# tenpy/cyten

Hardware: AMD Instinct MI355X
Metric: block-sparse tdot+SVD GFLOP/s (fp64) (higher is better)
Workload: dtype f64

## Files before the change

cyten_amd/csrc/blocked_qr.h:

```cpp
#pragma once
#include "common.h"

namespace cyb {

constexpr int NBK = 32;

struct BqrMat {
    double* Ac;
    int64_t ld;
    int32_t m, n, k;
    double* V;
    double* T;
    double* tau;
    double* scratch;
    int64_t scr_half;
    int32_t v_zeroed = 0;
    double* ctl = nullptr;
    double* parts = nullptr;
    double stop_rel2 = 0.0;
    int32_t reflect_always = 0;
};

size_t bqr_aux_bytes(int64_t m, int64_t n, int64_t ld, int64_t kc);
size_t bqr_carve(BqrMat& q, char* base, int64_t kc);

int bqr_strip_slots(int64_t rows);

int bqr_factor(cyb_ctx_t ctx, const std::vector<BqrMat>& mats);

struct BqrTarget {
    int32_t mat;
    double* C;
    int64_t ldc;
    int32_t kc;
};
int bqr_apply_q(cyb_ctx_t ctx, const std::vector<BqrMat>& mats, const std::vector<BqrTarget>& targets);

struct XposeDesc {
    const double* in;
    double* out;
    int64_t ldi, ldo;
    int32_t R, C, upper, rlim;
    int32_t plain, pad;
};
int xpose_batched(cyb_ctx_t ctx, const std::vector<XposeDesc>& descs);
struct EyeDesc {
    double* C;
    int64_t ld;
    int32_t m, kc;
    int32_t col0, pad;
};
int eye_cols_batched(cyb_ctx_t ctx, const std::vector<EyeDesc>& descs);

}
```

cyten_amd/csrc/blocked_qr.hip:

```cpp
#include "blocked_qr.h"

#include <algorithm>
#include <cstdlib>
#include <utility>

namespace cyb {
namespace {

#define GLOBAL_AS __attribute__((address_space(1)))
typedef GLOBAL_AS double* gp;
typedef const GLOBAL_AS double* gcp;
typedef double d4 __attribute__((ext_vector_type(4)));

constexpr int PNT = 512;
constexpr int PNW = PNT / 64;

__device__ __forceinline__ double wave_sum(double v)
{
#pragma unroll
    for (int o = 32; o > 0; o >>= 1) v += __shfl_xor(v, o);
    return v;
}

struct PanelDesc {
// ... 859 lines not shown
            }
        }
    }
    if constexpr (LA) {
        if (d.next_off) {
            asm volatile("s_waitcnt vmcnt(0)" ::: "memory");
            __syncthreads();
            if (tid == 0) {
                __builtin_amdgcn_fence(__ATOMIC_RELEASE, "agent");
                __hip_atomic_store(la_flags + (d.next_off - 1), la_tag, __ATOMIC_RELAXED, __HIP_MEMORY_SCOPE_AGENT);
            }
        }
    }
    if constexpr (FUSE_PANEL) {
        __shared__ PanelShared psh;
        if (d.next_off) {
            __syncthreads();
            const PanelDesc pd = *reinterpret_cast<const PanelDesc*>(reinterpret_cast<const char*>(descs) + d.next_off);
            panel_reg_body<RP_RPT_FUSED>(pd, psh, tid);
        }
    }
}

struct ChunkDesc {
    double* C;
    const double* V;
    const double* T;
    double* wpart;
    int64_t ldc, ldv;
    int32_t mr, nc, pw, transT;
    int32_t slot, n_slots, row0, step;
    const double* ctl;
    double* part_out;
};

__global__ void __launch_bounds__(ST_NT) strip_w1_kernel(const ChunkDesc* __restrict__ descs)
{
    __shared__ double part[ST_NW][NBK][ST_LS];
    const ChunkDesc d = descs[blockIdx.x];
    if (d.ctl) {
        const double stopped = *(gcp)d.ctl;
        if (stopped != 0.0 && (double)d.step >= stopped - 1.0) return;
    }
    const int tid = threadIdx.x, lane = tid & 63, wave = tid >> 6;
    const int x = lane & 15, kq = lane >> 4;
    gcp V = (gcp)d.V;
// ... 178 lines not shown
            for (int o = 32; o > 0; o >>= 1) nrm2 += __shfl_xor(nrm2, o);
            __syncthreads();
            if (lane == 0) W1s[0][wave] = nrm2;
            __syncthreads();
            if (tid == 0) {
                double t = 0.0;
#pragma unroll
                for (int w = 0; w < ST_NW; ++w) t += W1s[0][w];
                *(gp)d.part_out = t;
            }
        }
    }
}

inline size_t al256(size_t b) { return (b + 255) / 256 * 256; }

__global__ void __launch_bounds__(256) xpose_kernel(const XposeDesc* __restrict__ descs)
{
    __shared__ double tile[32][33];
    const XposeDesc d = descs[blockIdx.y];
    gcp in = (gcp)d.in;
    gp out = (gp)d.out;
    const int tx = threadIdx.x & 31, ty = threadIdx.x >> 5;
    if (d.plain) {
        const int64_t tot = (int64_t)d.R * d.C;
        for (int64_t e = (int64_t)blockIdx.x * 256 + threadIdx.x; e < tot; e += (int64_t)gridDim.x * 256) {
            const int64_t r = e / d.C, c = e % d.C;
            out[r * d.ldo + c] = in[r * d.ldi + c];
        }
        return;
    }
    const int tr = (d.R + 31) / 32, tc = (d.C + 31) / 32;
    for (int t = blockIdx.x; t < tr * tc; t += gridDim.x) {
        const int r0 = (t / tc) * 32, c0 = (t % tc) * 32;
        __syncthreads();
#pragma unroll
        for (int q = 0; q < 4; ++q) {
            const int c = c0 + ty + 8 * q, r = r0 + tx;
            tile[ty + 8 * q][tx] = (c < d.C && r < d.R) ? in[(int64_t)c * d.ldi + r] : 0.0;
        }
        __syncthreads();
#pragma unroll
        for (int q = 0; q < 4; ++q) {
            const int r = r0 + ty + 8 * q, c = c0 + tx;
            if (r < d.R && c < d.C) {
                double v = tile[tx][ty + 8 * q];
                if (d.upper && (r > c || r >= d.rlim)) v = 0.0;
                out[(int64_t)r * d.ldo + c] = v;
            }
        }
    }
}

__global__ void __launch_bounds__(256) eye_cols_kernel(const EyeDesc* __restrict__ descs)
{
    const EyeDesc d = descs[blockIdx.y];
    gp C = (gp)d.C;
    const int64_t tot = (int64_t)d.m * d.kc;
    for (int64_t e = (int64_t)blockIdx.x * 256 + threadIdx.x; e < tot; e += (int64_t)gridDim.x * 256) {
        const int64_t c = e / d.m, i = e % d.m;
        C[c * d.ld + i] = (i == c + d.col0) ? 1.0 : 0.0;
    }
}

}

int xpose_batched(cyb_ctx_t ctx, const std::vector<XposeDesc>& descs)
{
    if (descs.empty()) return CYB_OK;
    void* d = nullptr;
    CYB_TRY(ctx->upload(descs.data(), sizeof(XposeDesc) * descs.size(), &d));
    hipLaunchKernelGGL(xpose_kernel, dim3(helper_grid_x(descs.size()), (unsigned)descs.size()), dim3(256), 0, ctx->stream, static_cast<const XposeDesc*>(d));
    CYB_HIP(hipGetLastError());
// ... 462 lines not shown
    }
    if (last_rest >= 0) CYB_HIP(hipStreamWaitEvent(ctx->stream, ctx->ev_pool[2 * (size_t)last_rest + 1], 0));
    if (la_used) {
        unsigned int h_err = 0;
        CYB_HIP(hipMemcpyAsync(&h_err, la_flags + la_err, sizeof(unsigned int), hipMemcpyDeviceToHost, ctx->stream));
        CYB_HIP(hipStreamSynchronize(ctx->stream));
        if (h_err) {
            set_error("blocked QR: a look-ahead panel workgroup waited more than a second for its strip");
            return CYB_ERR_HIP;
        }
    }
    if (multi) {
        unsigned int h_err = 0;
        CYB_HIP(hipMemcpyAsync(&h_err, xbase + t_bytes, sizeof(unsigned int), hipMemcpyDeviceToHost, ctx->stream));
        CYB_HIP(hipStreamSynchronize(ctx->stream));
        if (h_err) {
            set_error("blocked QR: a workgroup of the multi-workgroup panel kernel waited more than a second for its partners");
            return CYB_ERR_HIP;
        }
    }
    return CYB_OK;
}

int bqr_apply_q(cyb_ctx_t ctx, const std::vector<BqrMat>& mats, const std::vector<BqrTarget>& targets)
{
    int max_pan = 0;
    for (const auto& t : targets) max_pan = std::max(max_pan, (mats[(size_t)t.mat].k + NBK - 1) / NBK);
    const bool strips = use_strips();
    struct Step {
        GemmStaged s1, s3;
        size_t off_sd = 0;
        unsigned n_sd = 0;
        size_t off_cd = 0;
        unsigned n_cd = 0;
    };
    const bool split = strips && strip_split_mode() != 0;
    double* wsplit = nullptr;
    if (split) {
        size_t n_ch = 0;
        for (const auto& t : targets) n_ch += (size_t)((t.kc + NBK - 1) / NBK) * (size_t)bqr_strip_slots(mats[(size_t)t.mat].m);
        void* w = nullptr;
        CYB_TRY(ctx->workspace(sizeof(double) * NBK * NBK * std::max<size_t>(n_ch, 1), &w, 4));
        wsplit = static_cast<double*>(w);
    }
    std::vector<Step> steps;
    std::vector<char> image;
    int chunk = 2;
    for (int c0 = max_pan - 1; c0 >= 0; c0 -= chunk, chunk *= 3) {
    const int c1 = std::max(-1, c0 - chunk);
    steps.clear();
    image.clear();
    for (int p = c0; p > c1; --p) {
        GemmBatch g1, g3;
        std::vector<StripDesc> sd;
        for (const auto& t : targets) {
            const BqrMat& q = mats[(size_t)t.mat];
            const int j0 = p * NBK;
            if (j0 >= q.k || t.kc <= 0) continue;
            const int pw = std::min(NBK, q.k - j0);
            const int64_t mr = q.m - j0;
            double* W1 = q.scratch + q.scr_half;
            CYB_REQUIRE((int64_t)NBK * t.kc <= q.scr_half, "bqr_apply_q: target wider than the carved scratch");
            const double* Vp = q.V + (size_t)j0 * q.ld + j0;
            double* Ct = t.C + j0;
            const double* Tp = q.T + (size_t)p * NBK * NBK;
            if (strips) {
                const size_t s_begin = sd.size();
                add_strips(sd, Ct, t.ldc, t.kc, Vp, q.ld, Tp, mr, pw, 0);
                if (q.ctl && q.stop_rel2 > 0.0)
                    for (size_t si = s_begin; si < sd.size(); ++si) {
                        sd[si].ctl = q.ctl;
                        sd[si].step = p;
                    }
                continue;
            }
            const int ns = w_split(mr);
            const int64_t chunk = ((mr + ns - 1) / ns + 15) / 16 * 16;
            const int32_t seg0 = (int32_t)g3.segs.size();
            for (int sidx = 0; sidx < ns; ++sidx) {
                const int64_t r0 = chunk * sidx, rows = std::min(chunk, mr - r0);
                if (rows <= 0) break;
                double* W2s = W1 + (size_t)sidx * q.scr_half;
                g1.add_post(W2s, pw, t.kc, t.kc, Vp + r0, q.ld, 1, Ct + r0, 1, t.ldc, rows, 1.0, 0.0, Tp, NBK, 1);
                g3.segs.push_back(cyb_gemm_seg{W2s, Vp, pw, 1, t.kc, q.ld, 1});
            }
            g3.probs.push_back(cyb_gemm_prob{Ct, t.kc, mr, t.ldc, seg0, (int32_t)g3.segs.size(), -1.0, 1.0});
        }
        if (g1.empty() && sd.empty()) continue;
        Step st;
        if (!g1.empty()) {
            CYB_TRY(g1.stage(ctx, image, st.s1));
            CYB_TRY(g3.stage(ctx, image, st.s3));
        }
        if (!sd.empty()) {
            sort_strips(sd);
            st.n_sd = (unsigned)sd.size();
            const size_t off = (image.size() + 255) / 256 * 256;
            image.resize(off + sizeof(StripDesc) * sd.size());
            memcpy(image.data() + off, sd.data(), sizeof(StripDesc) * sd.size());
            st.off_sd = off;
            std::vector<std::pair<int, int>> cnt;
            for (const auto& d : sd) cnt.push_back({d.mr, 1});
            const int step_ch = split ? choose_chunk_rows(cnt, ctx->n_cu) : 0;
            if (step_ch > 0) {
                std::vector<ChunkDesc> cd;
                make_chunks(sd, wsplit, step_ch, cd);
                st.n_cd = (unsigned)cd.size();
                const size_t offc = (image.size() + 255) / 256 * 256;
                image.resize(offc + sizeof(ChunkDesc) * cd.size());
                memcpy(image.data() + offc, cd.data(), sizeof(ChunkDesc) * cd.size());
                st.off_cd = offc;
            }
        }
        steps.push_back(st);
    }
    if (steps.empty()) continue;
    void* d_image = nullptr;
    CYB_TRY(ctx->upload(image.data(), image.size(), &d_image));
    for (const auto& st : steps) {
        if (st.n_cd) {
            const ChunkDesc* cdp = reinterpret_cast<const ChunkDesc*>(static_cast<char*>(d_image) + st.off_cd);
            hipLaunchKernelGGL(strip_w1_kernel, dim3(st.n_cd), dim3(ST_NT), 0, ctx->stream, cdp);
            hipLaunchKernelGGL(strip_apply_kernel<false>, dim3(st.n_cd), dim3(ST_NT), 0, ctx->stream, cdp);
            CYB_HIP(hipGetLastError());
        } else if (st.n_sd) {
            hipLaunchKernelGGL(reflector_strip_kernel<false>, dim3(st.n_sd), dim3(ST_NT), 0, ctx->stream,
                               reinterpret_cast<const StripDesc*>(static_cast<char*>(d_image) + st.off_sd), (int)st.n_sd,
                               static_cast<const PanelDesc*>(nullptr), static_cast<unsigned int*>(nullptr), 0u, 0);
            CYB_HIP(hipGetLastError());
        }
        CYB_TRY(gemm_launch_staged(ctx, st.s1, d_image));
        CYB_TRY(gemm_launch_staged(ctx, st.s3, d_image));
    }
    }
    return CYB_OK;
}

}
```

cyten_amd/csrc/svd_jacobi.hip:

```cpp
#include "blocked_qr.h"
#include "jacobi_engine.h"

#include <algorithm>
#include <cmath>
#include <cstdlib>

namespace cyb {
namespace {

#define GLOBAL_AS __attribute__((address_space(1)))
typedef GLOBAL_AS double* gp;
typedef const GLOBAL_AS double* gcp;

struct PrepDesc {
    const double* A;
    int64_t lda;
    int32_t m, n;
    double* W;
    double* J;
    int32_t nvp, lenp;
    int32_t transpose;
    int32_t pad;
    const double* shift;
};
// ... 90 lines not shown
    const double* sig_lq = nullptr;
};

__global__ void __launch_bounds__(256) row_norm_kernel(const PostDesc* __restrict__ descs)
{
    const PostDesc d = descs[blockIdx.y];
    gcp W = (gcp)d.W;
    const int lane = threadIdx.x & 63;
    for (int j = blockIdx.x * 4 + (threadIdx.x >> 6); j < d.nv; j += gridDim.x * 4) {
        double s = 0.0;
        for (int c = lane; c < d.len; c += 64) {
            const double v = W[(int64_t)j * d.lenp + c];
            s += v * v;
        }
#pragma unroll
        for (int o = 32; o > 0; o >>= 1) s += __shfl_xor(s, o);
        if (lane == 0) {
            const double o = d.sig_lq ? ((gcp)d.sig_lq)[j] : 0.0;
            ((gp)d.sig)[j] = (o > 0.0 && s > 0.0) ? o : sqrt(s);
        }
    }
}

__global__ void __launch_bounds__(256) rank_kernel(const PostDesc* __restrict__ descs)
{
    constexpr int CH = 2048;
    __shared__ double keys[CH];
    const PostDesc d = descs[blockIdx.y];
    gcp sig = (gcp)d.sig;
    const double shift = d.shift ? *(gcp)d.shift : 0.0;
    const int msk = d.cplx ? ~1 : ~0;
    const int per = (d.nv + (int)gridDim.x * 256 - 1) / ((int)gridDim.x * 256);
    for (int it = 0; it < per; ++it) {
        const int j = (it * (int)gridDim.x + (int)blockIdx.x) * 256 + (int)threadIdx.x;
        const bool mine = j < d.nv;
        const double sj = mine ? sig[j & msk] : 0.0;
        int r = 0;
        for (int k0 = 0; k0 < d.nv; k0 += CH) {
            const int kn = min(CH, d.nv - k0);
            __syncthreads();
            for (int k = threadIdx.x; k < kn; k += 256) keys[k] = sig[(k0 + k) & msk];
            __syncthreads();
            if (mine) {
                if (d.mode == 0) {
                    for (int k = 0; k < kn; ++k) {
                        const double sk = keys[k];
                        r += (sk > sj || (sk == sj && k0 + k < j)) ? 1 : 0;
                    }
                } else {
                    for (int k = 0; k < kn; ++k) {
                        const double sk = keys[k];
                        r += (sk < sj || (sk == sj && k0 + k < j)) ? 1 : 0;
                    }
                }
            }
        }
        if (mine) {
            d.rank[j] = r;
            d.S[r] = (d.mode == 0) ? sj : sj - shift;
        }
    }
}

__global__ void __launch_bounds__(256) write_factors_kernel(const PostDesc* __restrict__ descs)
{
    __shared__ double tile[32][33];
    __shared__ int rk[32];
    __shared__ double sc[32];
    const PostDesc d = descs[blockIdx.y];
    gcp W = (gcp)d.W;
    gcp J = (gcp)d.J;
    const int tx = threadIdx.x & 31, ty = threadIdx.x >> 5;
    double smax = 0.0;
    if (d.mode == 0) smax = ((gcp)d.S)[0];
    const double thresh = fmax(smax * 1e-280, 1e-300);

    const bool col_from_W = (d.mode == 1) || d.transposed;
    gcp csrc = col_from_W ? W : J;
    const int csrc_ld = col_from_W ? d.lenp : d.nvp;
    const int c_rows = col_from_W ? d.len : d.nv;
    gcp rsrc = col_from_W ? J : W;
    const int rsrc_ld = col_from_W ? d.nvp : d.lenp;
    const int r_cols = col_from_W ? d.nv : d.len;

// ... 272 lines not shown
        q.scratch = reinterpret_cast<double*>(base + o.scratch);
        q.n_null = reinterpret_cast<int32_t*>(base + o.nnull);
        q.null_scale = 0.0;
        q.cplx = cplx ? 1 : 0;
    }
    void* d_prep = nullptr;
    CYB_TRY(ctx->upload(prep.data(), sizeof(PrepDesc) * prep.size(), &d_prep));
    if (mode == 1) {
        void* d_nd = nullptr;
        CYB_TRY(ctx->upload(nd.data(), sizeof(NormDesc) * nd.size(), &d_nd));
        hipLaunchKernelGGL(fro_shift_kernel, dim3((unsigned)nmat), dim3(256), 0, st, static_cast<const NormDesc*>(d_nd));
    }
    hipLaunchKernelGGL(prep_kernel, dim3(64, (unsigned)nmat), dim3(256), 0, st, static_cast<const PrepDesc*>(d_prep));
    CYB_HIP(hipGetLastError());
    std::vector<int32_t> sweeps;
    const int jst = jacobi_orthogonalise(ctx, mats, 40, sweeps, cplx);
    if (info)
        for (int64_t b = 0; b < nmat; ++b) info[b] = sweeps[(size_t)b];
    if (jst != CYB_OK && jst != CYB_ERR_NOCONV) return jst;
    void* d_post = nullptr;
    CYB_TRY(ctx->upload(post.data(), sizeof(PostDesc) * post.size(), &d_post));
    const PostDesc* dp = static_cast<const PostDesc*>(d_post);
    hipLaunchKernelGGL(row_norm_kernel, dim3(helper_grid_x((size_t)nmat), (unsigned)nmat), dim3(256), 0, st, dp);
    hipLaunchKernelGGL(rank_kernel, dim3(8, (unsigned)nmat), dim3(256), 0, st, dp);
    hipLaunchKernelGGL(write_factors_kernel, dim3(helper_grid_x((size_t)nmat), (unsigned)nmat), dim3(256), 0, st, dp);
    if (mode == 0) hipLaunchKernelGGL(complete_null_kernel, dim3((unsigned)nmat), dim3(256), 0, st, dp);
    CYB_HIP(hipGetLastError());
    if (info) CYB_HIP(hipStreamSynchronize(st));
    return jst;
}


namespace {

struct RowsDesc {
    double* W;
    const double* sig;
    const int32_t* idx;
    double* buf;
    int32_t kp, k, cnt, pad;
    const int32_t* col;
};
__global__ void __launch_bounds__(256) gather_rows_kernel(const RowsDesc* __restrict__ descs)
{
    const RowsDesc d = descs[blockIdx.y];
    gcp W = (gcp)d.W;
    gp buf = (gp)d.buf;
// ... 228 lines not shown
#pragma unroll
        for (int o = 32; o > 0; o >>= 1) n2 += __shfl_xor(n2, o);
        if (lane == 0) ((gp)d.sigo)[d.idx[i]] = n2 > 0.0 ? f : 0.0;
        f = n2 > 0.0 ? f / sqrt(n2) : 0.0;
        for (int c = lane; c < d.kp; c += 64) Wc[(int64_t)i * d.kp + c] = c < d.k ? f * C[(int64_t)i * d.k + c] : 0.0;
    }
}

static int launch_row_moves(cyb_ctx_t ctx, const std::vector<RowMoveDesc>& v, bool jscatter = false)
{
    if (v.empty()) return CYB_OK;
    void* d = nullptr;
    CYB_TRY(ctx->upload(v.data(), sizeof(RowMoveDesc) * v.size(), &d));
    if (jscatter)
        hipLaunchKernelGGL(j_scatter_kernel, dim3(64, (unsigned)v.size()), dim3(256), 0, ctx->stream, static_cast<const RowMoveDesc*>(d));
    else
        hipLaunchKernelGGL(row_move_kernel, dim3(helper_grid_x(v.size()), (unsigned)v.size()), dim3(256), 0, ctx->stream, static_cast<const RowMoveDesc*>(d));
    CYB_HIP(hipGetLastError());
    return CYB_OK;
}

}

static int run_svd_qr(cyb_ctx_t ctx, int64_t nmat, const cyb_svd_desc* sd, int32_t* info, int flags, int32_t* rank_out)
{
    if (nmat == 0) return CYB_OK;
    const bool cplx = (flags & CYB_SVD_EMBEDDED_COMPLEX) != 0;
    hipStream_t st = ctx->stream;
    auto al = [](size_t b) { return (b + 255) / 256 * 256; };
    struct Lay {
        int m, n, k, L, kp;
        bool tall;
        size_t Ac, aux, W, J, sig, rank, thr, nnull, Cq, Fc, aux2, Cn, idx, Wc, Jc;
        size_t bad, Wq, aux3, Cq2, sig2;
        size_t stop;
        size_t sigo;
        size_t dev;
        bool lq = false;
        bool jrec = false;
        int r0 = 0;
        std::vector<int32_t> good0;
    };
    std::vector<Lay> lay((size_t)nmat);
    size_t off = 0;
    size_t sig_begin = off;
    for (int64_t b = 0; b < nmat; ++b) {
        Lay& l = lay[(size_t)b];
        l.m = (int)sd[b].m;
        l.n = (int)sd[b].n;
        l.k = std::min(l.m, l.n);
        l.L = std::max(l.m, l.n);
        l.kp = round_up(l.k, 64);
        l.tall = l.m >= l.n;
        l.sig = off;
        off += sizeof(double) * (size_t)l.kp;
    }
    for (int64_t b = 0; b < nmat; ++b) {
        lay[(size_t)b].thr = off;
        off += sizeof(double);
    }
    for (int64_t b = 0; b < nmat; ++b) {
        lay[(size_t)b].bad = off;
        off += sizeof(double);
    }
    for (int64_t b = 0; b < nmat; ++b) {
        lay[(size_t)b].dev = off;
        off += sizeof(double);
    }
    const size_t sig_bytes = off - sig_begin;
    off = al(off);
    for (int64_t b = 0; b < nmat; ++b) {
        Lay& l = lay[(size_t)b];
        auto take = [&](size_t bytes) {
            const size_t o = off;
            off += al(bytes);
            return o;
        };
        l.Ac = take(sizeof(double) * (size_t)l.L * l.k);
        l.aux = take(bqr_aux_bytes(l.L, l.k, l.L, l.k));
        l.stop = take(sizeof(double) * (size_t)(2 + (l.k + cyb::NBK - 1) / cyb::NBK * cyb::bqr_strip_slots(l.L)));
        l.W = take(sizeof(double) * (size_t)l.kp * l.kp);
        l.J = take(sizeof(double) * (size_t)l.kp * l.kp);
        l.rank = take(sizeof(int32_t) * (size_t)l.kp);
        l.nnull = take(sizeof(int32_t));
        l.Cq = take(sizeof(double) * (size_t)l.L * l.k);
        l.Fc = take(sizeof(double) * (size_t)l.k * l.k);
        l.aux2 = take(bqr_aux_bytes(l.k, l.k, l.k, l.k));
        l.Cn = take(sizeof(double) * (size_t)l.k * l.k);
        l.Wc = take(sizeof(double) * (size_t)l.kp * l.kp);
        l.Jc = take(sizeof(double) * (size_t)l.kp * l.kp);
        l.Wq = take(sizeof(double) * (size_t)l.kp * l.kp);
        l.aux3 = take(bqr_aux_bytes(l.k, l.k, l.kp, l.k));
        l.Cq2 = take(sizeof(double) * (size_t)l.k * l.k);
        l.sig2 = take(sizeof(double) * (size_t)l.kp);
        l.sigo = take(sizeof(double) * (size_t)l.kp);
    }
    const size_t idx_begin = off;
    for (int64_t b = 0; b < nmat; ++b) {
        lay[(size_t)b].idx = off;
        off += sizeof(int32_t) * (size_t)lay[(size_t)b].k;
    }
    off = al(off);
    void* ws = nullptr;
    CYB_TRY(ctx->workspace(off, &ws, 0));
    char* base = static_cast<char*>(ws);
    CYB_HIP(hipMemsetAsync(ws, 0, off, st));
    auto dp = [&](size_t o) { return reinterpret_cast<double*>(base + o); };

    std::vector<BqrMat> qm((size_t)nmat);
    std::vector<XposeDesc> x_in, x_r;
    std::vector<EyeDesc> eyeJ;
    std::vector<JMat> jm((size_t)nmat);
    for (int64_t b = 0; b < nmat; ++b) {
        const Lay& l = lay[(size_t)b];
        BqrMat& q = qm[(size_t)b];
        q.Ac = dp(l.Ac);
        q.ld = l.L;
        q.m = l.L;
        q.n = l.k;
        q.k = l.k;
        bqr_carve(q, base + l.aux, l.k);
        q.v_zeroed = 1;
        q.reflect_always = cplx ? 1 : 0;
        q.ctl = dp(l.stop);
        q.parts = dp(l.stop) + 2;
        q.stop_rel2 = ((double)l.L * 2.220446049250313e-16) * ((double)l.L * 2.220446049250313e-16);
        if (l.tall)
            x_in.push_back(XposeDesc{sd[b].A, q.Ac, sd[b].lda, l.L, l.n, l.m, 0, 0, 0, 0});
        else
            x_in.push_back(XposeDesc{sd[b].A, q.Ac, sd[b].lda, l.L, l.m, l.n, 0, 0, 1, 0});
        x_r.push_back(XposeDesc{q.Ac, dp(l.W), l.L, l.kp, l.k, l.k, 1, l.k, 0, 0});
        eyeJ.push_back(EyeDesc{dp(l.J), l.kp, l.kp, l.kp, 0, 0});
        JMat& j = jm[(size_t)b];
        j.W = dp(l.W);
        j.J = dp(l.J);
        j.nvp = l.kp;
        j.lenp = l.kp;
        j.nb = row_blocks(l.k, l.kp);
        j.nv = l.k;
        j.len = l.k;
        j.rec_j = 0;
        j.tol = 2.220446049250313e-16 * std::max(16.0, 4.0 * std::sqrt((double)l.k));
        j.thr2 = 0.0;
    }
    CYB_TRY(xpose_batched(ctx, x_in));
    CYB_TRY(bqr_factor(ctx, qm));
    CYB_TRY(xpose_batched(ctx, x_r));
    CYB_TRY(eye_cols_batched(ctx, eyeJ));
    std::vector<PostDesc> post((size_t)nmat);
    for (int64_t b = 0; b < nmat; ++b) {
        const Lay& l = lay[(size_t)b];
        PostDesc& q = post[(size_t)b];
        q.W = dp(l.W);
// ... 6 lines not shown
        q.mode = 0;
        q.sig = dp(l.sig);
        q.rank = reinterpret_cast<int32_t*>(base + l.rank);
        q.S = sd[b].S;
        q.U = l.tall ? nullptr : sd[b].U;
        q.ldu = sd[b].ldu;
        q.Vh = l.tall ? sd[b].Vh : nullptr;
        q.ldvh = sd[b].ldvh;
        q.shift = nullptr;
        q.scratch = nullptr;
        q.n_null = reinterpret_cast<int32_t*>(base + l.nnull);
        q.null_scale = 1.0;
        q.cplx = cplx ? 1 : 0;
    }
    void* d_post = nullptr;
    const PostDesc* dpost = nullptr;
    std::vector<double> h_sig(sig_bytes / sizeof(double));
    auto sig_of = [&](const Lay& l) { return h_sig.data() + (l.sig - sig_begin) / sizeof(double); };
    CYB_TRY(ctx->upload(post.data(), sizeof(PostDesc) * post.size(), &d_post));
    dpost = static_cast<const PostDesc*>(d_post);
    hipLaunchKernelGGL(row_norm_kernel, dim3(helper_grid_x((size_t)nmat), (unsigned)nmat), dim3(256), 0, st, dpost);
    CYB_HIP(hipGetLastError());
    CYB_TRY(ctx->d2h(h_sig.data(), base + sig_begin, sig_bytes));
    {
        std::vector<int32_t> idx_all;
        std::vector<size_t> idx_off((size_t)nmat, 0);
        for (int64_t b = 0; b < nmat; ++b) {
            Lay& l = lay[(size_t)b];
            const double* sg = sig_of(l);
            double fro2 = 0.0;
            for (int j = 0; j < l.k; ++j) fro2 += sg[j] * sg[j];
            const double sc = (double)l.L * 2.220446049250313e-16;
            const double thr2 = fro2 * sc * sc;
            jm[(size_t)b].thr2 = thr2;
            std::vector<int32_t> nul;
            for (int j = 0; j < l.k; ++j) {
                const double v = cplx ? std::max(sg[j & ~1], sg[std::min(j | 1, l.k - 1)]) : sg[j];
                (v * v > thr2 ? l.good0 : nul).push_back(j);
            }
            l.r0 = (int)l.good0.size();
            idx_off[(size_t)b] = idx_all.size();
            idx_all.insert(idx_all.end(), l.good0.begin(), l.good0.end());
            idx_all.insert(idx_all.end(), nul.begin(), nul.end());
        }
        static const bool no_lq = getenv("CYB_SVD_NOLQ") != nullptr;
        static const bool lq_always = getenv("CYB_SVD_LQ_ALWAYS") != nullptr;
// ... 271 lines not shown
                void* d = nullptr;
                CYB_TRY(ctx->upload(gath.data(), sizeof(RowsDesc) * gath.size(), &d));
                hipLaunchKernelGGL(gather_rows_kernel, dim3(64, (unsigned)gath.size()), dim3(256), 0, st,
                                   static_cast<const RowsDesc*>(d));
                CYB_HIP(hipGetLastError());
                CYB_TRY(bqr_factor(ctx, qm2));
            }
            CYB_TRY(eye_cols_batched(ctx, eyes));
            if (!tg2.empty()) CYB_TRY(bqr_apply_q(ctx, qm2, tg2));
            void* d = nullptr;
            if (!cols_all.empty()) {
                void* d_cols = nullptr;
                CYB_TRY(ctx->upload(cols_all.data(), sizeof(int32_t) * cols_all.size(), &d_cols));
                for (const auto& pr : lq_scat) scat[pr.first].col = static_cast<const int32_t*>(d_cols) + pr.second;
            }
            CYB_TRY(ctx->upload(scat.data(), sizeof(RowsDesc) * scat.size(), &d));
            hipLaunchKernelGGL(scatter_rows_kernel, dim3(64, (unsigned)scat.size()), dim3(256), 0, st,
                               static_cast<const RowsDesc*>(d));
            CYB_HIP(hipGetLastError());
        }
    }
    CYB_TRY(ctx->upload(post.data(), sizeof(PostDesc) * post.size(), &d_post));
    dpost = static_cast<const PostDesc*>(d_post);
    hipLaunchKernelGGL(rank_kernel, dim3(8, (unsigned)nmat), dim3(256), 0, st, dpost);
    hipLaunchKernelGGL(write_factors_kernel, dim3(helper_grid_x((size_t)nmat), (unsigned)nmat), dim3(256), 0, st, dpost);
    CYB_HIP(hipGetLastError());
    std::vector<JcqDesc> jc;
    std::vector<BqrTarget> tg;
    std::vector<XposeDesc> x_out;
    for (int64_t b = 0; b < nmat; ++b) {
        const Lay& l = lay[(size_t)b];
        jc.push_back(JcqDesc{dp(l.J), reinterpret_cast<const int32_t*>(base + l.rank), dp(l.Cq), l.L, l.kp, l.k});
        tg.push_back(BqrTarget{(int)b, dp(l.Cq), l.L, l.k});
        if (l.tall)
            x_out.push_back(XposeDesc{dp(l.Cq), sd[b].U, l.L, sd[b].ldu, l.m, l.k, 0, 0, 0, 0});
        else
            x_out.push_back(XposeDesc{dp(l.Cq), sd[b].Vh, l.L, sd[b].ldvh, l.k, l.n, 0, 0, 1, 0});
    }
    {
        void* d = nullptr;
        CYB_TRY(ctx->upload(jc.data(), sizeof(JcqDesc) * jc.size(), &d));
        hipLaunchKernelGGL(j_to_cq_kernel, dim3(helper_grid_x((size_t)nmat), (unsigned)nmat), dim3(256), 0, st, static_cast<const JcqDesc*>(d));
        CYB_HIP(hipGetLastError());
    }
    CYB_TRY(bqr_apply_q(ctx, qm, tg));
    CYB_TRY(xpose_batched(ctx, x_out));
    if (info) CYB_HIP(hipStreamSynchronize(st));
// ... 32 lines not shown
    for (const auto& d : nz) n_fit += cyb::svd_small_fits(d.m, d.n) ? 1 : 0;
    const bool embedded = (flags & CYB_SVD_EMBEDDED_COMPLEX) != 0;
    const bool use_small = !embedded && !no_small && (n_fit == nz.size() || n_fit >= 16);
    std::vector<cyb_svd_desc> tiny, small, large;
    std::vector<int64_t> idx_t, idx_s, idx_l;
    static const bool no_merge = getenv("CYB_SVD_NOMERGE") != nullptr;
    bool any_large = false;
    for (const auto& d : nz) any_large = any_large || (!no_qr && std::min(d.m, d.n) >= 48 && !(use_small && cyb::svd_small_fits(d.m, d.n)));
    (void)any_large;
    const int64_t large_min = embedded ? 1 : no_merge ? 48 : 2;
    for (size_t k = 0; k < nz.size(); ++k) {
        if (use_small && cyb::svd_small_fits(nz[k].m, nz[k].n)) {
            CYB_REQUIRE(nz[k].S, "svd block %lld: S is NULL", (long long)idx[k]);
            tiny.push_back(nz[k]);
            idx_t.push_back(idx[k]);
        } else if (!no_qr && std::min(nz[k].m, nz[k].n) >= large_min) {
            large.push_back(nz[k]);
            idx_l.push_back(idx[k]);
        } else {
            small.push_back(nz[k]);
            idx_s.push_back(idx[k]);
        }
    }
    std::vector<int32_t> inf_t(tiny.size()), inf_s(small.size()), inf_l(large.size());
    const int st_t = cyb::svd_small_batched(ctx, tiny.data(), (int64_t)tiny.size(), inf_t.data());
    if (st_t != CYB_OK && st_t != CYB_ERR_NOCONV) return st_t;
    if (info)
        for (size_t k = 0; k < tiny.size(); ++k) info[idx_t[k]] = inf_t[k];
    if (small.empty() && large.empty()) return st_t;
    std::vector<int32_t> rank_l(large.size());
    const int st_l = cyb::run_svd_qr(ctx, (int64_t)large.size(), large.data(), info ? inf_l.data() : nullptr, flags,
                                     rank_out ? rank_l.data() : nullptr);
    if (rank_out)
        for (size_t k = 0; k < large.size(); ++k) rank_out[idx_l[k]] = rank_l[k];
    if (st_l != CYB_OK && st_l != CYB_ERR_NOCONV) return st_l;
    const int st_s = cyb::run_jacobi(ctx, 0, (int64_t)small.size(), small.data(), nullptr, info ? inf_s.data() : nullptr);
    if (info) {
        for (size_t k = 0; k < small.size(); ++k) info[idx_s[k]] = inf_s[k];
        for (size_t k = 0; k < large.size(); ++k) info[idx_l[k]] = inf_l[k];
    }
    return st_s != CYB_OK ? st_s : (st_l != CYB_OK ? st_l : st_t);
}

static int eigh_batched_impl(cyb_ctx_t ctx, const cyb_eigh_desc* descs, int64_t n, int32_t* info, int flags = 0)
{
    CYB_REQUIRE(ctx, "cyb_eigh_batched_f64: ctx is NULL");
// ... 1 lines not shown
    std::vector<cyb_eigh_desc> nz;
    std::vector<int64_t> idx;
    for (int64_t b = 0; b < n; ++b) {
        if (info) info[b] = 0;
        if (descs[b].n > 0) {
            nz.push_back(descs[b]);
            idx.push_back(b);
        }
    }
    std::vector<int32_t> inf(nz.size());
    static const bool no_small = getenv("CYB_SVD_NOSMALL") != nullptr;
    const bool embedded = (flags & CYB_EIGH_EMBEDDED_COMPLEX) != 0;
    bool all_small = !no_small && !nz.empty() && !embedded;
    for (const auto& d : nz) all_small = all_small && d.n <= 64;
    const int st = all_small ? cyb::eigh_small_batched(ctx, nz.data(), (int64_t)nz.size(), inf.data())
                             : cyb::run_jacobi(ctx, 1, (int64_t)nz.size(), nullptr, nz.data(), info ? inf.data() : nullptr, embedded);
    if (info)
        for (size_t k = 0; k < nz.size(); ++k) info[idx[k]] = inf[k];
    return st;
}

static int svd_batched_ranged(cyb_ctx_t ctx, const cyb_svd_desc* descs, int64_t n, int32_t* info, int flags, int32_t* rank)
{
    std::vector<cyb::MatRef> refs;
    std::vector<int64_t> which;
    for (int64_t b = 0; b < n; ++b)
        if (descs[b].m > 0 && descs[b].n > 0 && descs[b].A) {
            refs.push_back(cyb::MatRef{descs[b].A, descs[b].lda, descs[b].m, descs[b].n});
            which.push_back(b);
        }
    std::vector<double> amax;
    CYB_TRY(cyb::matrix_amax(ctx, refs, amax));
    std::vector<cyb_svd_desc> mod;
    std::vector<void*> temps;
    std::vector<cyb::ScaleJob> pre, post;
    for (size_t k = 0; k < refs.size(); ++k) {
        const double sc = cyb::range_scale(amax[k]);
        if (sc == 1.0) continue;
        if (mod.empty()) mod.assign(descs, descs + n);
        cyb_svd_desc& d = mod[(size_t)which[k]];
        void* t = nullptr;
        CYB_HIP(hipMalloc(&t, sizeof(double) * (size_t)d.m * (size_t)d.n));
        temps.push_back(t);
        pre.push_back(cyb::ScaleJob{d.A, d.lda, static_cast<double*>(t), d.n, d.m, d.n, sc});
        d.A = static_cast<const double*>(t);
        d.lda = d.n;
// ... 93 lines not shown
```

Before: 5225.

## Fuse multi-panel Q application, defer range check, parallelize rank kernel

Adds a persistent kernel that applies a whole run of Householder panels to a column chunk in one launch. It software-pipelines V/C loads and uses MFMA for the W1, T·W1 and update steps, replacing the per-panel strip launches when enough chunks exist. It also stops applying panels past the early-stop point, and folds the amax range check into the transpose kernel so the SVD runs optimistically instead of doing a separate amax pass first. The rank kernel now splits each comparison loop across 16 lanes with a shuffle reduction. These add a retry path when scaling is needed and extra complexity in ordering and early-stop handling.

```diff
diff --git a/cyten_amd/csrc/blocked_qr.h b/cyten_amd/csrc/blocked_qr.h
--- a/cyten_amd/csrc/blocked_qr.h
+++ b/cyten_amd/csrc/blocked_qr.h
@@ -19,6 +19,7 @@
     double* parts = nullptr;
     double stop_rel2 = 0.0;
     int32_t reflect_always = 0;
+    int32_t n_pan_done = -1;
 };
 
 size_t bqr_aux_bytes(int64_t m, int64_t n, int64_t ld, int64_t kc);
@@ -42,6 +43,7 @@
     int64_t ldi, ldo;
     int32_t R, C, upper, rlim;
     int32_t plain, pad;
+    unsigned long long* amax = nullptr;
 };
 int xpose_batched(cyb_ctx_t ctx, const std::vector<XposeDesc>& descs);
 struct EyeDesc {
diff --git a/cyten_amd/csrc/blocked_qr.hip b/cyten_amd/csrc/blocked_qr.hip
--- a/cyten_amd/csrc/blocked_qr.hip
+++ b/cyten_amd/csrc/blocked_qr.hip
@@ -905,6 +905,234 @@
     }
 }
 
+struct ApplyDesc {
+    double* C;
+    const double* V;
+    const double* T;
+    const double* ctl;
+    int64_t ldc, ld;
+    int32_t m, k, nc;
+    int32_t p_lo, p_hi;
+    int32_t pad;
+};
+
+constexpr int AF_UN = 3;
+__global__ void __launch_bounds__(ST_NT) reflector_apply_fused_kernel(const ApplyDesc* __restrict__ descs)
+{
+    __shared__ double part[ST_NW][NBK][ST_LS];
+    __shared__ double W1s[NBK][ST_LS], W2s[NBK][ST_LS], Ps[NBK][ST_LS];
+    const ApplyDesc d = descs[blockIdx.x];
+    int p_hi = d.p_hi;
+    if (d.ctl) {
+        const double stopped = *(gcp)d.ctl;
+        if (stopped != 0.0) p_hi = min(p_hi, (int)stopped - 2);
+        p_hi = __builtin_amdgcn_readfirstlane(p_hi);
+    }
+    if (p_hi < d.p_lo) return;
+    const int tid0 = threadIdx.x;
+    const int nc = d.nc;
+    const int64_t ldv = d.ld, ldc = d.ldc;
+    static_assert(NBK * NBK == 2 * ST_NT, "two entries of T per thread");
+    static_assert(AF_UN * 4 * 64 <= NBK * ST_LS, "a wave's first batch of V fits its slice of part");
+    auto prefetch = [&](int p) {
+        int tid = tid0;
+        asm volatile("" : "+v"(tid));
+        const int lane = tid & 63, wave = tid >> 6;
+        const int x = lane & 15, kq = lane >> 4;
+        const int j0 = p * NBK, mr = d.m - j0, pw = min(NBK, d.k - j0);
+        gcp V = (gcp)d.V + (int64_t)j0 * ldv + j0;
+        gcp T = (gcp)d.T + (int64_t)p * (NBK * NBK);
+        Ps[tid / NBK][tid % NBK] = T[tid];
+        Ps[(tid + ST_NT) / NBK][tid % NBK] = T[tid + ST_NT];
+        const int64_t vo0 = (int64_t)(x < pw ? x : 0) * ldv, vo1 = (int64_t)(x + 16 < pw ? x + 16 : 0) * ldv;
+        double* stash = &part[wave][0][0] + lane;
+#pragma unroll
+        for (int u = 0; u < AF_UN; ++u) {
+            const int i = (wave + ST_NW * u) * 8 + 2 * kq;
+#pragma unroll
+            for (int h = 0; h < 2; ++h) {
+                const bool ok = i + h < mr;
+                const int ii = ok ? i + h : 0;
+                stash[(u * 4 + h) * 64] = ok ? V[vo0 + ii] : 0.0;
+                stash[(u * 4 + 2 + h) * 64] = ok ? V[vo1 + ii] : 0.0;
+            }
+        }
+    };
+    prefetch(p_hi);
+    for (int p = p_hi; p >= d.p_lo; --p) {
+        int tid = tid0;
+        asm volatile("" : "+v"(tid));
+        const int lane = tid & 63, wave = tid >> 6;
+        const int x = lane & 15, kq = lane >> 4;
+        const int j0 = p * NBK, mr = d.m - j0, pw = min(NBK, d.k - j0);
+        gcp V = (gcp)d.V + (int64_t)j0 * ldv + j0;
+        gp C = (gp)d.C + j0;
+        {
+            const int64_t vo0 = (int64_t)(x < pw ? x : 0) * ldv, vo1 = (int64_t)(x + 16 < pw ? x + 16 : 0) * ldv;
+            const int64_t co0 = (int64_t)(x < nc ? x : 0) * ldc, co1 = (int64_t)(x + 16 < nc ? x + 16 : 0) * ldc;
+            d4 acc[2][2];
+#pragma unroll
+            for (int i = 0; i < 2; ++i)
+#pragma unroll
+                for (int j = 0; j < 2; ++j) acc[i][j] = d4{0.0, 0.0, 0.0, 0.0};
+            const int nstep = (mr + 7) / 8;
+            double va[AF_UN][2][2], ca[AF_UN][2][2], vn[AF_UN][2][2], cn[AF_UN][2][2];
+#pragma unroll
+            for (int u = 0; u < AF_UN; ++u)
+#pragma unroll
+                for (int i = 0; i < 2; ++i)
+#pragma unroll
+                    for (int h = 0; h < 2; ++h) va[u][i][h] = (&part[wave][0][0] + lane)[(u * 4 + 2 * i + h) * 64];
+            auto load_c = [&](double (&c)[AF_UN][2][2], int s0) {
+#pragma unroll
+                for (int u = 0; u < AF_UN; ++u) {
+                    const int i = (s0 + ST_NW * u) * 8 + 2 * kq;
+#pragma unroll
+                    for (int h = 0; h < 2; ++h) {
+                        const bool ok = i + h < mr;
+                        const int ii = ok ? i + h : 0;
+                        c[u][0][h] = ok ? C[co0 + ii] : 0.0;
+                        c[u][1][h] = ok ? C[co1 + ii] : 0.0;
+                    }
+                }
+            };
+            auto load = [&](double (&v)[AF_UN][2][2], double (&c)[AF_UN][2][2], int s0) {
+#pragma unroll
+                for (int u = 0; u < AF_UN; ++u) {
+                    const int i = (s0 + ST_NW * u) * 8 + 2 * kq;
+#pragma unroll
+                    for (int h = 0; h < 2; ++h) {
+                        const bool ok = i + h < mr;
+                        const int ii = ok ? i + h : 0;
+                        v[u][0][h] = ok ? V[vo0 + ii] : 0.0;
+                        v[u][1][h] = ok ? V[vo1 + ii] : 0.0;
+                        c[u][0][h] = ok ? C[co0 + ii] : 0.0;
+                        c[u][1][h] = ok ? C[co1 + ii] : 0.0;
+                    }
+                }
+            };
+            if (wave < nstep) load_c(ca, wave);
+            for (int s0 = wave; s0 < nstep; s0 += ST_NW * AF_UN) {
+                const bool more = s0 + ST_NW * AF_UN < nstep;
+                if (more) load(vn, cn, s0 + ST_NW * AF_UN);
+#pragma unroll
+                for (int u = 0; u < AF_UN; ++u) {
+                    if (s0 + ST_NW * u < nstep) {
+#pragma unroll
+                        for (int h = 0; h < 2; ++h)
+#pragma unroll
+                            for (int i = 0; i < 2; ++i)
+#pragma unroll
+                                for (int j = 0; j < 2; ++j)
+                                    acc[i][j] = __builtin_amdgcn_mfma_f64_16x16x4f64(va[u][i][h], ca[u][j][h], acc[i][j], 0, 0, 0);
+                    }
+                }
+                if (more) {
+#pragma unroll
+                    for (int u = 0; u < AF_UN; ++u)
+#pragma unroll
+                        for (int i = 0; i < 2; ++i)
+#pragma unroll
+                            for (int h = 0; h < 2; ++h) {
+                                va[u][i][h] = vn[u][i][h];
+                                ca[u][i][h] = cn[u][i][h];
+                            }
+                }
+            }
+#pragma unroll
+            for (int i = 0; i < 2; ++i)
+#pragma unroll
+                for (int j = 0; j < 2; ++j)
+#pragma unroll
+                    for (int r = 0; r < 4; ++r) part[wave][i * 16 + kq + 4 * r][j * 16 + x] = acc[i][j][r];
+        }
+        __syncthreads();
+        for (int e = tid; e < NBK * NBK; e += ST_NT) {
+            const int a = e / NBK, c = e % NBK;
+            double t = 0.0;
+#pragma unroll
+            for (int w = 0; w < ST_NW; ++w) t += part[w][a][c];
+            W1s[a][c] = t;
+        }
+        __syncthreads();
+        if (wave < 4) {
+            const int ta = wave >> 1, tc = wave & 1;
+            d4 acc = d4{0.0, 0.0, 0.0, 0.0};
+#pragma unroll
+            for (int kk = 0; kk < NBK / 4; ++kk)
+                acc = __builtin_amdgcn_mfma_f64_16x16x4f64(Ps[ta * 16 + x][4 * kk + kq], W1s[4 * kk + kq][tc * 16 + x], acc, 0, 0, 0);
+#pragma unroll
+            for (int r = 0; r < 4; ++r) W2s[ta * 16 + kq + 4 * r][tc * 16 + x] = acc[r];
+        }
+        __syncthreads();
+        {
+            double w2[2][NBK / 4];
+#pragma unroll
+            for (int ct = 0; ct < 2; ++ct)
+#pragma unroll
+                for (int kk = 0; kk < NBK / 4; ++kk) w2[ct][kk] = -W2s[4 * kk + kq][ct * 16 + x];
+            int64_t vcol[NBK / 4], ccol[2][4];
+#pragma unroll
+            for (int kk = 0; kk < NBK / 4; ++kk) vcol[kk] = (int64_t)(4 * kk + kq < pw ? 4 * kk + kq : 0) * ldv;
+#pragma unroll
+            for (int ct = 0; ct < 2; ++ct)
+#pragma unroll
+                for (int r = 0; r < 4; ++r) {
+                    const int c = ct * 16 + kq + 4 * r;
+                    ccol[ct][r] = (int64_t)(c < nc ? c : 0) * ldc;
+                }
+            const int ntile = (mr + 15) / 16;
+            struct Tile {
+                double v[NBK / 4];
+                d4 c[2];
+            };
+            auto load = [&](Tile& t, int rt) {
+                const int i = rt * 16 + x;
+                const bool ok = i < mr;
+                const int ii = ok ? i : 0;
+#pragma unroll
+                for (int kk = 0; kk < NBK / 4; ++kk) t.v[kk] = ok ? V[vcol[kk] + ii] : 0.0;
+#pragma unroll
+                for (int ct = 0; ct < 2; ++ct)
+#pragma unroll
+                    for (int r = 0; r < 4; ++r) t.c[ct][r] = C[ccol[ct][r] + ii];
+            };
+            auto finish = [&](Tile& t, int rt) {
+#pragma unroll
+                for (int kk = 0; kk < NBK / 4; ++kk) {
+                    t.c[0] = __builtin_amdgcn_mfma_f64_16x16x4f64(w2[0][kk], t.v[kk], t.c[0], 0, 0, 0);
+                    t.c[1] = __builtin_amdgcn_mfma_f64_16x16x4f64(w2[1][kk], t.v[kk], t.c[1], 0, 0, 0);
+                }
+                const int i = rt * 16 + x;
+                if (i < mr) {
+#pragma unroll
+                    for (int ct = 0; ct < 2; ++ct)
+#pragma unroll
+                        for (int r = 0; r < 4; ++r)
+                            if (ct * 16 + kq + 4 * r < nc) C[ccol[ct][r] + i] = t.c[ct][r];
+                }
+            };
+            Tile t0, t1, t2;
+            if (wave < ntile) load(t0, wave);
+            if (wave + ST_NW < ntile) load(t1, wave + ST_NW);
+            for (int rt = wave; rt < ntile; rt += 3 * ST_NW) {
+                if (rt + 2 * ST_NW < ntile) load(t2, rt + 2 * ST_NW);
+                finish(t0, rt);
+                if (rt + ST_NW < ntile) {
+                    if (rt + 3 * ST_NW < ntile) load(t0, rt + 3 * ST_NW);
+                    finish(t1, rt + ST_NW);
+                }
+                if (rt + 2 * ST_NW < ntile) {
+                    if (rt + 4 * ST_NW < ntile) load(t1, rt + 4 * ST_NW);
+                    finish(t2, rt + 2 * ST_NW);
+                }
+            }
+        }
+        if (p > d.p_lo) prefetch(p - 1);
+        __syncthreads();
+    }
+}
+
 struct ChunkDesc {
     double* C;
     const double* V;
@@ -1129,33 +1357,43 @@
     gcp in = (gcp)d.in;
     gp out = (gp)d.out;
     const int tx = threadIdx.x & 31, ty = threadIdx.x >> 5;
+    unsigned long long amx = 0;
     if (d.plain) {
         const int64_t tot = (int64_t)d.R * d.C;
         for (int64_t e = (int64_t)blockIdx.x * 256 + threadIdx.x; e < tot; e += (int64_t)gridDim.x * 256) {
             const int64_t r = e / d.C, c = e % d.C;
-            out[r * d.ldo + c] = in[r * d.ldi + c];
-        }
-        return;
-    }
-    const int tr = (d.R + 31) / 32, tc = (d.C + 31) / 32;
-    for (int t = blockIdx.x; t < tr * tc; t += gridDim.x) {
-        const int r0 = (t / tc) * 32, c0 = (t % tc) * 32;
-        __syncthreads();
-#pragma unroll
-        for (int q = 0; q < 4; ++q) {
-            const int c = c0 + ty + 8 * q, r = r0 + tx;
-            tile[ty + 8 * q][tx] = (c < d.C && r < d.R) ? in[(int64_t)c * d.ldi + r] : 0.0;
-        }
-        __syncthreads();
-#pragma unroll
-        for (int q = 0; q < 4; ++q) {
-            const int r = r0 + ty + 8 * q, c = c0 + tx;
-            if (r < d.R && c < d.C) {
-                double v = tile[tx][ty + 8 * q];
-                if (d.upper && (r > c || r >= d.rlim)) v = 0.0;
-                out[(int64_t)r * d.ldo + c] = v;
-            }
-        }
+            const double v = in[r * d.ldi + c];
+            amx = max(amx, (unsigned long long)__double_as_longlong(fabs(v)));
+            out[r * d.ldo + c] = v;
+        }
+    } else {
+        const int tr = (d.R + 31) / 32, tc = (d.C + 31) / 32;
+        for (int t = blockIdx.x; t < tr * tc; t += gridDim.x) {
+            const int r0 = (t / tc) * 32, c0 = (t % tc) * 32;
+            __syncthreads();
+#pragma unroll
+            for (int q = 0; q < 4; ++q) {
+                const int c = c0 + ty + 8 * q, r = r0 + tx;
+                const double v = (c < d.C && r < d.R) ? in[(int64_t)c * d.ldi + r] : 0.0;
+                amx = max(amx, (unsigned long long)__double_as_longlong(fabs(v)));
+                tile[ty + 8 * q][tx] = v;
+            }
+            __syncthreads();
+#pragma unroll
+            for (int q = 0; q < 4; ++q) {
+                const int r = r0 + ty + 8 * q, c = c0 + tx;
+                if (r < d.R && c < d.C) {
+                    double v = tile[tx][ty + 8 * q];
+                    if (d.upper && (r > c || r >= d.rlim)) v = 0.0;
+                    out[(int64_t)r * d.ldo + c] = v;
+                }
+            }
+        }
+    }
+    if (d.amax) {
+#pragma unroll
+        for (int o = 32; o > 0; o >>= 1) amx = max(amx, __shfl_xor(amx, o));
+        if ((threadIdx.x & 63) == 0 && amx != 0) atomicMax(d.amax, amx);
     }
 }
 
@@ -1664,10 +1902,21 @@
     return CYB_OK;
 }
 
+static int apply_fuse_mode()
+{
+    static const int v = getenv("CYB_QR_APPLY_PERSTEP") ? 0 : getenv("CYB_QR_APPLY_FUSED") ? 2 : 1;
+    return v;
+}
+
 int bqr_apply_q(cyb_ctx_t ctx, const std::vector<BqrMat>& mats, const std::vector<BqrTarget>& targets)
 {
+    auto n_pan_all = [&](const BqrTarget& t) { return t.kc <= 0 ? 0 : (mats[(size_t)t.mat].k + NBK - 1) / NBK; };
+    auto n_pan = [&](const BqrTarget& t) {
+        const BqrMat& q = mats[(size_t)t.mat];
+        return q.n_pan_done >= 0 ? std::min(n_pan_all(t), (int)q.n_pan_done) : n_pan_all(t);
+    };
     int max_pan = 0;
-    for (const auto& t : targets) max_pan = std::max(max_pan, (mats[(size_t)t.mat].k + NBK - 1) / NBK);
+    for (const auto& t : targets) max_pan = std::max(max_pan, n_pan(t));
     const bool strips = use_strips();
     struct Step {
         GemmStaged s1, s3;
@@ -1675,6 +1924,8 @@
         unsigned n_sd = 0;
         size_t off_cd = 0;
         unsigned n_cd = 0;
+        size_t off_ad = 0;
+        unsigned n_ad = 0;
     };
     const bool split = strips && strip_split_mode() != 0;
     double* wsplit = nullptr;
@@ -1685,20 +1936,73 @@
         CYB_TRY(ctx->workspace(sizeof(double) * NBK * NBK * std::max<size_t>(n_ch, 1), &w, 4));
         wsplit = static_cast<double*>(w);
     }
+    std::vector<int> step_ch((size_t)max_pan, 0), run_lo((size_t)max_pan, -1);
+    if (strips) {
+        const int mode = apply_fuse_mode();
+        std::vector<char> whole((size_t)max_pan, 0);
+        for (int p = 0; p < max_pan; ++p) {
+            std::vector<std::pair<int, int>> cnt;
+            int64_t n_sd = 0;
+            for (const auto& t : targets)
+                if (p < n_pan_all(t)) {
+                    cnt.push_back({(int)(mats[(size_t)t.mat].m - p * NBK), (t.kc + NBK - 1) / NBK});
+                    n_sd += cnt.back().second;
+                }
+            step_ch[(size_t)p] = split ? choose_chunk_rows(cnt, ctx->n_cu) : 0;
+            whole[(size_t)p] = step_ch[(size_t)p] == 0 && (mode == 2 || (mode == 1 && n_sd * 4 > (int64_t)ctx->n_cu * 3));
+        }
+        for (int p = max_pan - 1; p >= 0; --p) {
+            if (!whole[(size_t)p]) continue;
+            int lo = p;
+            while (lo > 0 && whole[(size_t)lo - 1]) --lo;
+            if (lo < p) run_lo[(size_t)p] = lo;
+            p = lo;
+        }
+    }
     std::vector<Step> steps;
     std::vector<char> image;
     int chunk = 2;
-    for (int c0 = max_pan - 1; c0 >= 0; c0 -= chunk, chunk *= 3) {
-    const int c1 = std::max(-1, c0 - chunk);
+    for (int c0 = max_pan - 1; c0 >= 0;) {
     steps.clear();
     image.clear();
-    for (int p = c0; p > c1; --p) {
+    int p = c0;
+    for (int left = chunk; p >= 0 && left > 0; --left) {
+        if (run_lo[(size_t)p] >= 0) {
+            const int p_lo = run_lo[(size_t)p];
+            std::vector<ApplyDesc> ad;
+            std::vector<int64_t> work;
+            for (const auto& t : targets) {
+                const int np = n_pan(t);
+                if (p_lo >= np) continue;
+                const BqrMat& q = mats[(size_t)t.mat];
+                CYB_REQUIRE((int64_t)NBK * t.kc <= q.scr_half, "bqr_apply_q: target wider than the carved scratch");
+                const int hi = std::min(p, np - 1);
+                int64_t w = 0;
+                for (int s = p_lo; s <= hi; ++s) w += q.m - (int64_t)s * NBK;
+                for (int64_t cc = 0; cc < t.kc; cc += NBK) {
+                    ad.push_back(ApplyDesc{t.C + (size_t)cc * t.ldc, q.V, q.T, q.ctl && q.stop_rel2 > 0.0 ? q.ctl : nullptr, t.ldc, q.ld, q.m,
+                                           q.k, (int32_t)std::min<int64_t>(NBK, t.kc - cc), p_lo, hi, 0});
+                    work.push_back(w);
+                }
+            }
+            std::vector<size_t> ord(ad.size());
+            for (size_t i = 0; i < ord.size(); ++i) ord[i] = i;
+            std::stable_sort(ord.begin(), ord.end(), [&](size_t a, size_t b) { return work[a] > work[b]; });
+            Step st;
+            st.n_ad = (unsigned)ad.size();
+            st.off_ad = (image.size() + 255) / 256 * 256;
+            image.resize(st.off_ad + sizeof(ApplyDesc) * ad.size());
+            for (size_t i = 0; i < ord.size(); ++i) memcpy(image.data() + st.off_ad + sizeof(ApplyDesc) * i, &ad[ord[i]], sizeof(ApplyDesc));
+            steps.push_back(st);
+            p = p_lo - 1;
+            continue;
+        }
         GemmBatch g1, g3;
         std::vector<StripDesc> sd;
         for (const auto& t : targets) {
             const BqrMat& q = mats[(size_t)t.mat];
             const int j0 = p * NBK;
-            if (j0 >= q.k || t.kc <= 0) continue;
+            if (p >= n_pan(t)) continue;
             const int pw = std::min(NBK, q.k - j0);
             const int64_t mr = q.m - j0;
             double* W1 = q.scratch + q.scr_half;
@@ -1728,6 +2032,7 @@
             }
             g3.probs.push_back(cyb_gemm_prob{Ct, t.kc, mr, t.ldc, seg0, (int32_t)g3.segs.size(), -1.0, 1.0});
         }
+        --p;
         if (g1.empty() && sd.empty()) continue;
         Step st;
         if (!g1.empty()) {
@@ -1741,12 +2046,10 @@
             image.resize(off + sizeof(StripDesc) * sd.size());
             memcpy(image.data() + off, sd.data(), sizeof(StripDesc) * sd.size());
             st.off_sd = off;
-            std::vector<std::pair<int, int>> cnt;
-            for (const auto& d : sd) cnt.push_back({d.mr, 1});
-            const int step_ch = split ? choose_chunk_rows(cnt, ctx->n_cu) : 0;
-            if (step_ch > 0) {
+            const int step_rows = step_ch[(size_t)(p + 1)];
+            if (step_rows > 0) {
                 std::vector<ChunkDesc> cd;
-                make_chunks(sd, wsplit, step_ch, cd);
+                make_chunks(sd, wsplit, step_rows, cd);
                 st.n_cd = (unsigned)cd.size();
                 const size_t offc = (image.size() + 255) / 256 * 256;
                 image.resize(offc + sizeof(ChunkDesc) * cd.size());
@@ -1756,10 +2059,18 @@
         }
         steps.push_back(st);
     }
+    c0 = p;
+    chunk *= 3;
     if (steps.empty()) continue;
     void* d_image = nullptr;
     CYB_TRY(ctx->upload(image.data(), image.size(), &d_image));
     for (const auto& st : steps) {
+        if (st.n_ad) {
+            hipLaunchKernelGGL(reflector_apply_fused_kernel, dim3(st.n_ad), dim3(ST_NT), 0, ctx->stream,
+                               reinterpret_cast<const ApplyDesc*>(static_cast<char*>(d_image) + st.off_ad));
+            CYB_HIP(hipGetLastError());
+            continue;
+        }
         if (st.n_cd) {
             const ChunkDesc* cdp = reinterpret_cast<const ChunkDesc*>(static_cast<char*>(d_image) + st.off_cd);
             hipLaunchKernelGGL(strip_w1_kernel, dim3(st.n_cd), dim3(ST_NT), 0, ctx->stream, cdp);
diff --git a/cyten_amd/csrc/svd_jacobi.hip b/cyten_amd/csrc/svd_jacobi.hip
--- a/cyten_amd/csrc/svd_jacobi.hip
+++ b/cyten_amd/csrc/svd_jacobi.hip
@@ -136,6 +136,7 @@
     }
 }
 
+template <int G>
 __global__ void __launch_bounds__(256) rank_kernel(const PostDesc* __restrict__ descs)
 {
     constexpr int CH = 2048;
@@ -144,9 +145,10 @@
     gcp sig = (gcp)d.sig;
     const double shift = d.shift ? *(gcp)d.shift : 0.0;
     const int msk = d.cplx ? ~1 : ~0;
-    const int per = (d.nv + (int)gridDim.x * 256 - 1) / ((int)gridDim.x * 256);
-    for (int it = 0; it < per; ++it) {
-        const int j = (it * (int)gridDim.x + (int)blockIdx.x) * 256 + (int)threadIdx.x;
+    const int per_wg = 256 / G;
+    const int sub = (int)threadIdx.x % G;
+    for (int j0 = (int)blockIdx.x * per_wg; j0 < d.nv; j0 += (int)gridDim.x * per_wg) {
+        const int j = j0 + (int)threadIdx.x / G;
         const bool mine = j < d.nv;
         const double sj = mine ? sig[j & msk] : 0.0;
         int r = 0;
@@ -157,23 +159,32 @@
             __syncthreads();
             if (mine) {
                 if (d.mode == 0) {
-                    for (int k = 0; k < kn; ++k) {
+                    for (int k = sub; k < kn; k += G) {
                         const double sk = keys[k];
                         r += (sk > sj || (sk == sj && k0 + k < j)) ? 1 : 0;
                     }
                 } else {
-                    for (int k = 0; k < kn; ++k) {
+                    for (int k = sub; k < kn; k += G) {
                         const double sk = keys[k];
                         r += (sk < sj || (sk == sj && k0 + k < j)) ? 1 : 0;
                     }
                 }
             }
         }
-        if (mine) {
+#pragma unroll
+        for (int o = G / 2; o > 0; o >>= 1) r += __shfl_xor(r, o);
+        if (mine && sub == 0) {
             d.rank[j] = r;
             d.S[r] = (d.mode == 0) ? sj : sj - shift;
         }
     }
+}
+
+static void launch_rank(hipStream_t st, const PostDesc* dp, int64_t nmat)
+{
+    static const bool serial = getenv("CYB_SVD_RANK_SERIAL") != nullptr;
+    if (serial) hipLaunchKernelGGL(rank_kernel<1>, dim3(8, (unsigned)nmat), dim3(256), 0, st, dp);
+    else hipLaunchKernelGGL(rank_kernel<16>, dim3(helper_grid_x((size_t)nmat), (unsigned)nmat), dim3(256), 0, st, dp);
 }
 
 __global__ void __launch_bounds__(256) write_factors_kernel(const PostDesc* __restrict__ descs)
@@ -492,7 +503,7 @@
     CYB_TRY(ctx->upload(post.data(), sizeof(PostDesc) * post.size(), &d_post));
     const PostDesc* dp = static_cast<const PostDesc*>(d_post);
     hipLaunchKernelGGL(row_norm_kernel, dim3(helper_grid_x((size_t)nmat), (unsigned)nmat), dim3(256), 0, st, dp);
-    hipLaunchKernelGGL(rank_kernel, dim3(8, (unsigned)nmat), dim3(256), 0, st, dp);
+    launch_rank(st, dp, nmat);
     hipLaunchKernelGGL(write_factors_kernel, dim3(helper_grid_x((size_t)nmat), (unsigned)nmat), dim3(256), 0, st, dp);
     if (mode == 0) hipLaunchKernelGGL(complete_null_kernel, dim3((unsigned)nmat), dim3(256), 0, st, dp);
     CYB_HIP(hipGetLastError());
@@ -767,6 +778,9 @@
 
 }
 
+constexpr int kSvdRangeDeferred = 1 << 30;
+constexpr int kSvdRangeRetry = -1000;
+
 static int run_svd_qr(cyb_ctx_t ctx, int64_t nmat, const cyb_svd_desc* sd, int32_t* info, int flags, int32_t* rank_out)
 {
     if (nmat == 0) return CYB_OK;
@@ -781,6 +795,8 @@
         size_t stop;
         size_t sigo;
         size_t dev;
+        size_t ctl;
+        size_t amx;
         bool lq = false;
         bool jrec = false;
         int r0 = 0;
@@ -812,6 +828,14 @@
         lay[(size_t)b].dev = off;
         off += sizeof(double);
     }
+    for (int64_t b = 0; b < nmat; ++b) {
+        lay[(size_t)b].ctl = off;
+        off += 2 * sizeof(double);
+    }
+    for (int64_t b = 0; b < nmat; ++b) {
+        lay[(size_t)b].amx = off;
+        off += sizeof(double);
+    }
     const size_t sig_bytes = off - sig_begin;
     off = al(off);
     for (int64_t b = 0; b < nmat; ++b) {
@@ -823,7 +847,7 @@
         };
         l.Ac = take(sizeof(double) * (size_t)l.L * l.k);
         l.aux = take(bqr_aux_bytes(l.L, l.k, l.L, l.k));
-        l.stop = take(sizeof(double) * (size_t)(2 + (l.k + cyb::NBK - 1) / cyb::NBK * cyb::bqr_strip_slots(l.L)));
+        l.stop = take(sizeof(double) * (size_t)((l.k + cyb::NBK - 1) / cyb::NBK * cyb::bqr_strip_slots(l.L)));
         l.W = take(sizeof(double) * (size_t)l.kp * l.kp);
         l.J = take(sizeof(double) * (size_t)l.kp * l.kp);
         l.rank = take(sizeof(int32_t) * (size_t)l.kp);
@@ -867,13 +891,14 @@
         bqr_carve(q, base + l.aux, l.k);
         q.v_zeroed = 1;
         q.reflect_always = cplx ? 1 : 0;
-        q.ctl = dp(l.stop);
-        q.parts = dp(l.stop) + 2;
+        q.ctl = dp(l.ctl);
+        q.parts = dp(l.stop);
         q.stop_rel2 = ((double)l.L * 2.220446049250313e-16) * ((double)l.L * 2.220446049250313e-16);
         if (l.tall)
             x_in.push_back(XposeDesc{sd[b].A, q.Ac, sd[b].lda, l.L, l.n, l.m, 0, 0, 0, 0});
         else
             x_in.push_back(XposeDesc{sd[b].A, q.Ac, sd[b].lda, l.L, l.m, l.n, 0, 0, 1, 0});
+        if (flags & kSvdRangeDeferred) x_in.back().amax = reinterpret_cast<unsigned long long*>(base + l.amx);
         x_r.push_back(XposeDesc{q.Ac, dp(l.W), l.L, l.kp, l.k, l.k, 1, l.k, 0, 0});
         eyeJ.push_back(EyeDesc{dp(l.J), l.kp, l.kp, l.kp, 0, 0});
         JMat& j = jm[(size_t)b];
@@ -926,6 +951,20 @@
     hipLaunchKernelGGL(row_norm_kernel, dim3(helper_grid_x((size_t)nmat), (unsigned)nmat), dim3(256), 0, st, dpost);
     CYB_HIP(hipGetLastError());
     CYB_TRY(ctx->d2h(h_sig.data(), base + sig_begin, sig_bytes));
+    if (flags & kSvdRangeDeferred)
+        for (int64_t b = 0; b < nmat; ++b) {
+            double amax;
+            memcpy(&amax, reinterpret_cast<const char*>(h_sig.data()) + (lay[(size_t)b].amx - sig_begin), sizeof(double));
+            if (range_scale(amax) != 1.0) return kSvdRangeRetry;
+        }
+    {
+        static const bool all_panels = getenv("CYB_QR_APPLY_ALLPANELS") != nullptr;
+        for (int64_t b = 0; b < nmat && !all_panels; ++b) {
+            const Lay& l = lay[(size_t)b];
+            const double stopped = h_sig[(l.ctl - sig_begin) / sizeof(double)];
+            qm[(size_t)b].n_pan_done = stopped != 0.0 ? (int32_t)stopped - 1 : (l.k + cyb::NBK - 1) / cyb::NBK;
+        }
+    }
     {
         std::vector<int32_t> idx_all;
         std::vector<size_t> idx_off((size_t)nmat, 0);
@@ -1243,7 +1282,7 @@
     }
     CYB_TRY(ctx->upload(post.data(), sizeof(PostDesc) * post.size(), &d_post));
     dpost = static_cast<const PostDesc*>(d_post);
-    hipLaunchKernelGGL(rank_kernel, dim3(8, (unsigned)nmat), dim3(256), 0, st, dpost);
+    launch_rank(st, dpost, nmat);
     hipLaunchKernelGGL(write_factors_kernel, dim3(helper_grid_x((size_t)nmat), (unsigned)nmat), dim3(256), 0, st, dpost);
     CYB_HIP(hipGetLastError());
     std::vector<JcqDesc> jc;
@@ -1322,6 +1361,7 @@
             idx_s.push_back(idx[k]);
         }
     }
+    if ((flags & cyb::kSvdRangeDeferred) && (!tiny.empty() || !small.empty())) return cyb::kSvdRangeRetry;
     std::vector<int32_t> inf_t(tiny.size()), inf_s(small.size()), inf_l(large.size());
     const int st_t = cyb::svd_small_batched(ctx, tiny.data(), (int64_t)tiny.size(), inf_t.data());
     if (st_t != CYB_OK && st_t != CYB_ERR_NOCONV) return st_t;
@@ -1369,6 +1409,11 @@
 
 static int svd_batched_ranged(cyb_ctx_t ctx, const cyb_svd_desc* descs, int64_t n, int32_t* info, int flags, int32_t* rank)
 {
+    static const bool precheck = getenv("CYB_SVD_RANGE_PRECHECK") != nullptr;
+    if (!precheck) {
+        const int st = svd_batched_impl(ctx, descs, n, info, flags | cyb::kSvdRangeDeferred, rank);
+        if (st != cyb::kSvdRangeRetry) return st;
+    }
     std::vector<cyb::MatRef> refs;
     std::vector<int64_t> which;
     for (int64_t b = 0; b < n; ++b)
```

Result: slower. 5151 (-1.4%).
